# ethz-asl/laser_slam

Measured on AMD Instinct MI355X. Metric: scans_per_sec, higher is better.
Workload: dtype f32

## Files before the change

laser_slam_amd/csrc/lsgpu_icp.hip:

```cpp
#include <cstring>
#include <cmath>
#include <cstdio>
#include <cstdlib>
#include <string>
#include <vector>
#include <chrono>
#include <system_error>
#include <thread>
#include <utility>

#include <dlfcn.h>

#include <hip/hip_runtime.h>
#include <rccl/rccl.h>

#include "../../include/lsgpu_icp.h"
#include "lsgpu_grid.hip.h"
#include "lsgpu_tuning.h"
#include "lsgpu_policy.h"
#include "lsgpu_knn.hip.h"
#include "lsgpu_knn_k.hip.h"
#include "lsgpu_snf.hip.h"
#include "lsgpu_max_density.hip.h"
#include "lsgpu_cone.hip.h"
// ... 218 lines not shown
  DevBuf<double> amb_val;

  DevBuf<SsnSeg> ssn_seg_a, ssn_seg_b;
  DevBuf<int> ssn_axis_a, ssn_axis_b;
  DevBuf<uint32_t> ssn_seg_fb;
  DevBuf<SegBlock> ssn_blocktab;
  DevBuf<uint32_t> ssn_seg_of, ssn_box_pts, ssn_box_base, ssn_keep, ssn_out_pos, ssn_bb, ssn_bounds_ws;
  DevBuf<float> ssn_box_normal, ssn_draws;
  DevBuf<uint32_t> gs_e[2], gs_k[6];
  DevBuf<GsBlock> gs_tab;
  DevBuf<GsSegBlocks> gs_sblk;
  DevBuf<uint32_t> gs_hist;
  DevBuf<GsMedian> gs_cand, gs_median;
  DevBuf<uint32_t> gs_cand_blk, gs_cand_n, gs_cl, gs_err;
  DevBuf<uint2> gs_rng;
  uint32_t* h_gs_err = nullptr;
  int64_t gs_plan_n = -1;
  int gs_plan_levels = -1;
  std::vector<uint32_t> gs_lvl_first, gs_lvl_blocks;
  DevBuf<float4> flt_in, flt_in2, flt_ref, flt_rd;
  DevBuf<float4> vgf_out;
  DevBuf<float> flt_nrm;
  bool cuts_on = false;
  lsgpu_chain_cuts cuts{};
  DevBuf<uint32_t> cut_blk;
  DevBuf<float4> cut_ref;
  bool md_on = false;
  lsgpu_max_density_config md_cfg{};
  DevBuf<float> dens, dens_io;
  DevBuf<MdStat> md_stat;
// ... 335 lines not shown
  for (auto& e : h->knn_events) { (void)hipEventDestroy(e.a); (void)hipEventDestroy(e.b); (void)hipEventDestroy(e.c); (void)hipEventDestroy(e.d); (void)hipEventDestroy(e.e); }
  if (h->ev0) (void)hipEventDestroy(h->ev0);
  if (h->ev1) (void)hipEventDestroy(h->ev1);
  if (h->ev_state) (void)hipEventDestroy(h->ev_state);
  if (h->ev_tail) (void)hipEventDestroy(h->ev_tail);
  if (h->cone_done) (void)hipEventDestroy(h->cone_done);
  if (h->cone_occ_ready) (void)hipEventDestroy(h->cone_occ_ready);
  for (auto& e : h->ev_pay) if (e) (void)hipEventDestroy(e);
  if (h->pin) (void)hipHostFree(h->pin);
  if (h->h_price) (void)hipHostFree(h->h_price);
  if (h->h_cone_occ) (void)hipHostFree(h->h_cone_occ);
  if (h->h_gs_err) (void)hipHostFree(h->h_gs_err);
  for (auto& bf : h->gs_e) bf.release();
  for (auto& bf : h->gs_k) bf.release();
  h->gs_tab.release(); h->gs_sblk.release(); h->gs_hist.release(); h->gs_cand.release(); h->gs_median.release();
  h->gs_cand_blk.release(); h->gs_cand_n.release(); h->gs_cl.release(); h->gs_err.release(); h->gs_rng.release();
  if (h->draws_pinned) (void)hipHostFree(h->draws_pinned);
  if (h->copy_done) (void)hipEventDestroy(h->copy_done);
  if (h->ref_up_done) (void)hipEventDestroy(h->ref_up_done);
  if (h->draws_done) (void)hipEventDestroy(h->draws_done);
  if (h->draws_first_done) (void)hipEventDestroy(h->draws_first_done);
  if (h->draw_stream) { (void)hipStreamSynchronize(h->draw_stream); (void)hipStreamDestroy(h->draw_stream); }
  if (h->side_done) (void)hipEventDestroy(h->side_done);
  if (h->side_stream) { (void)hipStreamSynchronize(h->side_stream); (void)hipStreamDestroy(h->side_stream); }
  if (h->copy_stream) (void)hipStreamDestroy(h->copy_stream);
  if (h->stream) (void)hipStreamDestroy(h->stream);
  delete h;
}

}

// ... 1131 lines not shown
        HIPC(hipMemcpyAsync(h->gs_tab.p, tab.data(), tab.size() * sizeof(GsBlock), hipMemcpyHostToDevice, h->stream));
        HIPC(hipMemcpyAsync(h->gs_sblk.p, sblk.data(), sblk.size() * sizeof(GsSegBlocks), hipMemcpyHostToDevice, h->stream));
        HIPC(hipStreamSynchronize(h->stream));
      }
      h->gs_plan_n = n; h->gs_plan_levels = glevels;
    }
    const size_t nseg_g = (size_t)1 << glevels;
    int cap = 1;
    for (uint32_t v : h->gs_lvl_blocks) cap = std::max(cap, (int)v);
    for (auto& bf : h->gs_e) HIPC(bf.reserve(n));
    for (auto& bf : h->gs_k) HIPC(bf.reserve(n));
    HIPC(h->gs_hist.reserve(4 * 256 * (nseg_g + 1))); HIPC(h->gs_median.reserve(nseg_g)); HIPC(h->gs_cand_n.reserve(2 * nseg_g + 2));
    const size_t cand_room = std::max<size_t>(nseg_g / 2, 1) * kGsCandRoom;
    HIPC(h->gs_cand.reserve(cand_room)); HIPC(h->gs_cand_blk.reserve(cand_room));
    HIPC(h->gs_cl.reserve((size_t)2 * cap)); HIPC(h->gs_err.reserve(8)); HIPC(h->gs_rng.reserve(2 * nseg_g + 2));
    HIPC(h->ssn_axis_a.reserve(nseg_g)); HIPC(h->ssn_axis_b.reserve(nseg_g));
    if (!h->h_gs_err) HIPC(hipHostMalloc((void**)&h->h_gs_err, 64, hipHostMallocDefault));
    uint32_t* cand_n[2] = {h->gs_cand_n.p, h->gs_cand_n.p + nseg_g + 1};
    uint32_t* sig_cur = reinterpret_cast<uint32_t*>(h->ssn_axis_a.p);
    uint32_t* sig_nxt = reinterpret_cast<uint32_t*>(h->ssn_axis_b.p);
    GsSet in, out;
    in.e = h->gs_e[0].p; out.e = h->gs_e[1].p;
    for (int d = 0; d < 3; ++d) { in.k[d] = h->gs_k[d].p; out.k[d] = h->gs_k[3 + d].p; }
    uint2* rng_cur = h->gs_rng.p;
    uint2* rng_nxt = h->gs_rng.p + nseg_g + 1;
    uint32_t* gh1[2] = {h->gs_hist.p, h->gs_hist.p + 256 * (nseg_g + 1)};
    uint32_t* gh2[2] = {h->gs_hist.p + 2 * 256 * (nseg_g + 1), h->gs_hist.p + 3 * 256 * (nseg_g + 1)};
    hipLaunchKernelGGL(k_gs_init, dim3(nblk(n)), dim3(256), 0, h->stream, src, (int)n, in, out.e, (const SsnSeg*)cur, (const uint32_t*)h->ssn_bb.p, rng_cur,
                       gh1[0], gh2[0], cand_n[0], sig_cur, h->gs_err.p);
    for (int L = 0; L < glevels; ++L) {
      const int ns = 1 << L, nb = (int)h->gs_lvl_blocks[L], par = L & 1;
      const GsBlock* tab = h->gs_tab.p + h->gs_lvl_first[L];
      const GsSegBlocks* sblk = h->gs_sblk.p + (ns - 1);
      hipLaunchKernelGGL(k_gs_hist<1>, dim3(nb), dim3(256), 0, h->stream, tab, cur, (const uint2*)rng_cur, in, gh1[par], gh2[par], h->gs_err.p);
      hipLaunchKernelGGL(k_gs_hist<2>, dim3(nb), dim3(256), 0, h->stream, tab, cur, (const uint2*)rng_cur, in, gh1[par], gh2[par], h->gs_err.p);
      const uint32_t lvl_cap = (uint32_t)std::min<size_t>(cand_room / (size_t)ns, (size_t)1 << 22);
      hipLaunchKernelGGL(k_gs_collect, dim3(nb), dim3(256), 0, h->stream, tab, cur, (const uint2*)rng_cur, (const uint32_t*)sig_cur, in,
                         (const uint32_t*)gh1[par], (const uint32_t*)gh2[par], cand_n[par], h->gs_cand.p, h->gs_cand_blk.p, lvl_cap, h->gs_cl.p);
      hipLaunchKernelGGL(k_gs_select, dim3(ns), dim3(L < 3 ? 1024 : 256), 0, h->stream, sblk, src, cur, (const uint32_t*)sig_cur, gh1[par], gh2[par],
                         gh1[par ^ 1], gh2[par ^ 1], cand_n[par], (const GsMedian*)h->gs_cand.p, (const uint32_t*)h->gs_cand_blk.p, lvl_cap, h->gs_cl.p,
                         h->gs_cl.p + cap, h->gs_median.p, nxt, sig_nxt, cand_n[par ^ 1], rng_nxt, h->gs_err.p);
      hipLaunchKernelGGL(k_gs_part, dim3(nb), dim3(kGsPartThreads), 0, h->stream, tab, cur, (const uint32_t*)sig_cur, in, out,
                         (const GsMedian*)h->gs_median.p, (const uint32_t*)(h->gs_cl.p + cap), (const SsnSeg*)nxt, rng_nxt, h->gs_err.p);
      std::swap(in, out);
      std::swap(cur, nxt);
      std::swap(sig_cur, sig_nxt);
      std::swap(rng_cur, rng_nxt);
    }
    idx = in.e;
    root_sig = sig_cur;
    HIPC(hipGetLastError());
  } else if (glevels > 0) {
    const size_t nseg_g = (size_t)1 << glevels;
    const int cap = (int)(n / kSegTile + (int64_t)(nseg_g / 2) + 2);
    HIPC(h->lane.scratch->vals_alt.reserve(n));
    HIPC(h->ssn_axis_a.reserve(nseg_g)); HIPC(h->ssn_axis_b.reserve(nseg_g)); HIPC(h->ssn_seg_fb.reserve(nseg_g));
    HIPC(h->ssn_blocktab.reserve((size_t)cap)); HIPC(h->lane.scratch->sort_hist.reserve((size_t)256 * cap + 256 + 4));
    uint32_t* keyA = reinterpret_cast<uint32_t*>(h->lane.scratch->keys.p);
    uint32_t* keyB = keyA + n;
// ... 38 lines not shown
    uint32_t* idx_rw = const_cast<uint32_t*>(idx);
    if (root_max == 8192)
      hipLaunchKernelGGL(k_ssn_tree<8192>, dim3(1 << glevels), dim3(1024), 0, h->stream, src, idx_rw, cur, knn, levels - glevels, h->ssn_seg_of.p, nxt, root_axis, root_sig);
    else if (root_max == 4096)
      hipLaunchKernelGGL(k_ssn_tree<4096>, dim3(1 << glevels), dim3(512), 0, h->stream, src, idx_rw, cur, knn, levels - glevels, h->ssn_seg_of.p, nxt, root_axis, root_sig);
    else
      hipLaunchKernelGGL(k_ssn_tree<2048>, dim3(1 << glevels), dim3(256), 0, h->stream, src, idx_rw, cur, knn, levels - glevels, h->ssn_seg_of.p, nxt, root_axis, root_sig);
    std::swap(cur, nxt);
  }
  if (levels == 0) {
    hipLaunchKernelGGL(k_ssn_keys, dim3(nblk(n)), dim3(256), 0, h->stream, src, (int)n, (const uint32_t*)nullptr,
                       (const uint32_t*)nullptr, cur, knn, h->lane.scratch->keys.p, h->lane.scratch->vals.p);
    HIPC(hipMemsetAsync(h->ssn_seg_of.p, 0, (size_t)n * 4, h->stream));
    idx = h->lane.scratch->vals.p;
  }
  hipLaunchKernelGGL(k_ssn_boxes, dim3((int)((nseg + 127) / 128)), dim3(128), 0, h->stream, src, idx, cur, (int)nseg,
                     h->ssn_box_normal.p, h->ssn_box_pts.p);
  HIPC(hipGetLastError());
  int rc = scan_u32(h, h->ssn_box_pts.p, h->ssn_box_base.p, nseg);
  if (rc) return rc;
  rc = ahead->ready(first_draw + (size_t)n);
  if (rc) return rc;
  hipLaunchKernelGGL(k_ssn_select, dim3(nblk(n)), dim3(256), 0, h->stream, (int)n, idx, h->ssn_seg_of.p, cur,
                     h->ssn_box_pts.p, h->ssn_box_base.p, h->ssn_draws.p + first_draw, ratio, h->ssn_keep.p);
  rc = scan_u32(h, h->ssn_keep.p, h->ssn_out_pos.p, (size_t)n, false,  true);
  if (rc == LSGPU_OK) {
    hipLaunchKernelGGL(k_ssn_emit, dim3(nblk(n)), dim3(256), 0, h->stream, src, (int)n,
                       h->ssn_box_normal.p, h->ssn_keep.p, h->ssn_out_pos.p, out_xyz1, out_nrm);
  }
  uint32_t n_draws = 0, kept = 0;
  if (rc == LSGPU_OK)
    rc = scan_totals(h, h->ssn_box_pts.p, h->ssn_box_base.p, nseg, h->ssn_keep.p, h->ssn_out_pos.p, (size_t)n, &n_draws, &kept,
// ... 1624 lines not shown
```

laser_slam_amd/csrc/lsgpu_ssn.hip.h:

```cpp
#pragma once
#include "lsgpu_common.hip.h"
#include "lsgpu_box_normal.h"
#include "lsgpu_segsort.hip.h"
#include "lsgpu_chain_cut.hip.h"

namespace lsgpu {

struct SsnSeg {
  uint32_t start, count;
  float lo[3], hi[3];
};
constexpr int kSsnMaxKnn = 32;

__device__ __forceinline__ uint32_t float_order_key(float f) {
  uint32_t u = __float_as_uint(f);
  if (u == 0x80000000u) u = 0u;
  return (u & 0x80000000u) ? ~u : (u | 0x80000000u);
}
__device__ __forceinline__ float float_from_order_key(uint32_t k) {
  return __uint_as_float((k & 0x80000000u) ? (k & 0x7FFFFFFFu) : ~k);
}

__device__ __forceinline__ float coord_of(const float4& p, int d) { return d == 0 ? p.x : (d == 1 ? p.y : p.z); }

// ... 237 lines not shown
  const SsnSeg sg = segs[s];
  uint32_t kept = 0;
  if (sg.count > 0) {
    float n[3];
    const uint32_t* bi = idx + sg.start;
    if (boxnormal::box_normal((int)sg.count, [&](int i, int d) { return coord_of(p[bi[i]], d); }, n)) {
      kept = sg.count;
      box_normal[3 * (size_t)s + 0] = n[0];
      box_normal[3 * (size_t)s + 1] = n[1];
      box_normal[3 * (size_t)s + 2] = n[2];
    }
  }
  box_pts[s] = kept;
}

__global__ __launch_bounds__(256) void k_ssn_select(int n, const uint32_t* __restrict__ idx,
                                                    const uint32_t* __restrict__ seg_of,
                                                    const SsnSeg* __restrict__ segs,
                                                    const uint32_t* __restrict__ box_pts,
                                                    const uint32_t* __restrict__ box_base,
                                                    const float* __restrict__ draws, float ratio,
                                                    uint32_t* __restrict__ keep) {
  const int pos = blockIdx.x * 256 + threadIdx.x;
  if (pos >= n) return;
  const uint32_t s = seg_of[pos];
  uint32_t k = 0;
  if (box_pts[s]) {
    const float r = draws[box_base[s] + ((uint32_t)pos - segs[s].start)];
    k = r < ratio ? 1u : 0u;
  }
// ... 138 lines not shown
```

laser_slam_amd/csrc/lsgpu_ssn_select.hip.h:

```cpp
#pragma once
#include "lsgpu_ssn.hip.h"
#include "lsgpu_ssn_tree.hip.h"

namespace lsgpu {

#ifdef LSGPU_KNN_STATS
#define LSGPU_SEL_T(n) do { if (gridDim.x == 1 && threadIdx.x == 0) g_tree_dbg[n] = (unsigned long long)clock64(); } while (0)
#else
#define LSGPU_SEL_T(n) do { } while (0)
#endif

constexpr uint32_t kGsTile = 2048u;
constexpr int kGsPartThreads = 512;
constexpr uint32_t kGsCandCap = 2048u;
constexpr uint32_t kGsCandRoom = 16384u;
constexpr uint32_t kGsNoAxis = 0xFFu;
constexpr uint32_t kGsSelBlocks = 8192u;

struct GsSet {
  uint32_t* e;
  uint32_t* k[3];
};
__device__ __forceinline__ uint32_t* gs_k(const GsSet& g, int d) { return d == 0 ? g.k[0] : d == 1 ? g.k[1] : g.k[2]; }

struct GsBlock {
  uint32_t first, count;
  uint32_t seg;
  uint32_t seg_start, seg_count;
  uint32_t fb, nb;
  uint32_t pad;
};
struct GsSegBlocks { uint32_t fb, nb, start, count; };

struct GsMedian { uint32_t ka, k1, k2, e; };

__host__ __device__ __forceinline__ uint32_t gs_sig_push(uint32_t sig, uint32_t a) {
  const uint32_t o1 = sig & 0xFFu, o2 = (sig >> 8) & 0xFFu, o3 = (sig >> 16) & 0xFFu;
  if (o1 == a) return sig;
  const uint32_t r2 = o2 == a ? o3 : o2;
  return a | (o1 << 8) | (r2 << 16) | 0xFF000000u;
}
__device__ __forceinline__ void gs_other_axes(uint32_t sig, uint32_t a, uint32_t& x1, uint32_t& x2) {
  const uint32_t o1 = sig & 0xFFu, o2 = (sig >> 8) & 0xFFu, o3 = (sig >> 16) & 0xFFu;
  if (o1 == a) { x1 = o2; x2 = o3; }
  else { x1 = o1; x2 = o2 == a ? o3 : o2; }
}
__device__ __forceinline__ bool gs_less(uint32_t ka, uint32_t k1, uint32_t k2, uint32_t e, const GsMedian& m) {
  return ka != m.ka ? ka < m.ka : k1 != m.k1 ? k1 < m.k1 : k2 != m.k2 ? k2 < m.k2 : e < m.e;
}
// ... 32 lines not shown
  const uint32_t total = fbs[ns];
  for (uint32_t sg = threadIdx.x; sg < ns; sg += 1024u)
    sblk[(ns - 1u) + sg] = GsSegBlocks{fbs[sg], fbs[sg + 1u] - fbs[sg], sc[sg].x, sc[sg].y};
  GsBlock* __restrict__ t = tab + lvl.first[L];
  for (uint32_t j = threadIdx.x; j < total; j += 1024u) {
    uint32_t lo = 0u, hi = ns;
    while (hi - lo > 1u) { const uint32_t mid = (lo + hi) >> 1; if (fbs[mid] <= j) lo = mid; else hi = mid; }
    const uint32_t k = j - fbs[lo], st = sc[lo].x, c = sc[lo].y;
    const uint32_t off = k * kGsTile;
    t[j] = GsBlock{st + off, min(kGsTile, c - off), lo, st, c, fbs[lo], fbs[lo + 1u] - fbs[lo], 0u};
  }
}

__global__ __launch_bounds__(256) void k_gs_init(const float4* __restrict__ p, int n, GsSet out, uint32_t* __restrict__ other_e,
                                                 const SsnSeg* __restrict__ root, const uint32_t* __restrict__ bb,
                                                 uint2* __restrict__ rng, uint32_t* __restrict__ gh1_root,
                                                 uint32_t* __restrict__ gh2_root, uint32_t* __restrict__ cand_n_root,
                                                 uint32_t* __restrict__ sig_root, uint32_t* __restrict__ err) {
  const int i = blockIdx.x * 256 + threadIdx.x;
  if (blockIdx.x == 0) {
    gh1_root[threadIdx.x] = 0u; gh2_root[threadIdx.x] = 0u;
    if (threadIdx.x < 8) err[threadIdx.x] = 0u;
    if (threadIdx.x == 0) {
      const int a = ssn_cut_axis(root[0]); rng[0] = make_uint2(bb[a], bb[3 + a]);
      cand_n_root[0] = 0u; sig_root[0] = 0xFFFFFFFFu;
    }
  }
  if (i >= n) return;
  const float4 v = p[i];
  out.e[i] = (uint32_t)i; other_e[i] = (uint32_t)i;
  out.k[0][i] = float_order_key(v.x); out.k[1][i] = float_order_key(v.y); out.k[2][i] = float_order_key(v.z);
}

struct GsCut { int a; uint32_t klo, khi; float xlo, scale; };
__device__ __forceinline__ GsCut gs_cut(const SsnSeg& sg, const uint2 rng ) {
  GsCut c;
  c.a = ssn_cut_axis(sg);
  c.klo = rng.x; c.khi = rng.y >= rng.x ? rng.y : rng.x;
  c.xlo = float_from_order_key(c.klo);
  const float ext = float_from_order_key(c.khi) - c.xlo;
  c.scale = ext > 0.f ? 65536.0f / ext : 0.f;
  return c;
}
__device__ __forceinline__ uint32_t gs_bin16(const GsCut& c, uint32_t k) {
  const float t = (float_from_order_key(k) - c.xlo) * c.scale;
  return (uint32_t)fminf(fmaxf(t, 0.f), 65535.f);
}

__device__ __forceinline__ void gs_find_bin(const uint32_t* __restrict__ gh, uint32_t target, uint32_t* sh ,
                                            uint32_t& bin, uint32_t& below) {
  const int lane = threadIdx.x & 63, w = threadIdx.x >> 6;
  const bool act = threadIdx.x < 256u;
  const uint32_t tot = act ? gh[threadIdx.x] : 0u;
  const uint32_t incl = wave_scan_incl_u32(tot, lane);
  if (threadIdx.x == 0) { sh[4] = 0xFFFFFFFFu; sh[5] = 0u; }
  if (act && lane == 63) sh[w] = incl;
  __syncthreads();
  uint32_t before = 0u;
  for (int ww = 0; ww < w && ww < 4; ++ww) before += sh[ww];
  const uint32_t excl = before + incl - tot;
  if (act && tot != 0u && excl <= target && target < excl + tot) { sh[4] = threadIdx.x; sh[5] = excl; }
  __syncthreads();
  bin = sh[4]; below = sh[5];
  __syncthreads();
}

template <int PASS>
__global__ __launch_bounds__(256) void k_gs_hist(const GsBlock* __restrict__ tab, const SsnSeg* __restrict__ segs,
                                                 const uint2* __restrict__ rng, GsSet in, uint32_t* __restrict__ gh1,
                                                 uint32_t* __restrict__ gh2, uint32_t* __restrict__ err) {
  __shared__ uint32_t hist[256];
  __shared__ uint32_t sh[8];
  hist[threadIdx.x] = 0u;
  const GsBlock sb = tab[blockIdx.x];
  const GsCut c = gs_cut(segs[sb.seg], rng[sb.seg]);
  const uint32_t* __restrict__ ka = gs_k(in, c.a);
  uint32_t mb1 = 0u, below1 = 0u;
  if (PASS == 2) gs_find_bin(gh1 + (size_t)sb.seg * 256u, sb.seg_count - sb.seg_count / 2u, sh, mb1, below1);
  else __syncthreads();
  bool bad = PASS == 2 && mb1 == 0xFFFFFFFFu;
  for (uint32_t j = threadIdx.x; j < sb.count; j += 256u) {
    const uint32_t k = ka[sb.first + j];
    bad = bad || k < c.klo || k > c.khi;
    const uint32_t b16 = gs_bin16(c, k), b1 = b16 >> 8;
    if (PASS == 1) atomicAdd(&hist[b1], 1u);
    else if (b1 == mb1) atomicAdd(&hist[b16 & 255u], 1u);
  }
  if (bad) { err[0] = 1u; err[1] = 1u; err[2] = sb.seg; }
  __syncthreads();
  const uint32_t v = hist[threadIdx.x];
  if (v) atomicAdd(&(PASS == 1 ? gh1 : gh2)[(size_t)sb.seg * 256u + threadIdx.x], v);
}

__global__ __launch_bounds__(256) void k_gs_collect(const GsBlock* __restrict__ tab, const SsnSeg* __restrict__ segs,
                                                    const uint2* __restrict__ rng,
                                                    const uint32_t* __restrict__ sig, GsSet in, const uint32_t* __restrict__ gh1,
                                                    const uint32_t* __restrict__ gh2,
                                                    uint32_t* __restrict__ cand_n, GsMedian* __restrict__ cand,
                                                    uint32_t* __restrict__ cand_blk, uint32_t cap ,
                                                    uint32_t* __restrict__ cl) {
  __shared__ uint32_t ws[4];
  __shared__ uint32_t sh[8];
  const GsBlock sb = tab[blockIdx.x];
  const GsCut c = gs_cut(segs[sb.seg], rng[sb.seg]);
  const uint32_t leftn = sb.seg_count - sb.seg_count / 2u;
  uint32_t mb1, below1, mb2, below2;
  gs_find_bin(gh1 + (size_t)sb.seg * 256u, leftn, sh, mb1, below1);
  gs_find_bin(gh2 + (size_t)sb.seg * 256u, leftn - below1, sh, mb2, below2);
  uint32_t x1, x2;
  gs_other_axes(sig[sb.seg], (uint32_t)c.a, x1, x2);
  const uint32_t* __restrict__ ka = gs_k(in, c.a);
  uint32_t left = 0u;
  const int lane = threadIdx.x & 63;
  for (uint32_t j0 = 0; j0 < sb.count; j0 += 256u) {
    const uint32_t j = j0 + threadIdx.x;
    const bool live = j < sb.count;
    const uint32_t i = sb.first + (live ? j : 0u);
    const uint32_t k = live ? ka[i] : 0u;
    const uint32_t b16 = gs_bin16(c, k), b1 = b16 >> 8, b2 = b16 & 255u;
    const bool is_cand = live && b1 == mb1 && b2 == mb2;
    if (live && (b1 < mb1 || (b1 == mb1 && b2 < mb2))) ++left;
    const unsigned long long m = __ballot(is_cand);
    if (m != 0ull) {
      uint32_t base = 0u;
      if (lane == 0) base = atomicAdd(&cand_n[sb.seg], (uint32_t)__popcll(m));
      base = (uint32_t)__shfl((int)base, 0);
      const uint32_t slot = base + (uint32_t)__popcll(m & ((1ull << lane) - 1ull));
      if (is_cand && slot < cap) {
        GsMedian md;
        md.ka = k; md.e = in.e[i];
        md.k1 = x1 != kGsNoAxis ? gs_k(in, (int)x1)[i] : 0u;
        md.k2 = x2 != kGsNoAxis ? gs_k(in, (int)x2)[i] : 0u;
        cand[(size_t)sb.seg * cap + slot] = md;
        cand_blk[(size_t)sb.seg * cap + slot] = blockIdx.x;
// ... 3 lines not shown
  left = wave_sum_u32(left);
  if ((threadIdx.x & 63) == 0) ws[threadIdx.x >> 6] = left;
  __syncthreads();
  if (threadIdx.x == 0) cl[blockIdx.x] = ws[0] + ws[1] + ws[2] + ws[3];
}

__global__ __launch_bounds__(1024) void k_gs_select(const GsSegBlocks* __restrict__ sblk, const float4* __restrict__ p,
                                                   const SsnSeg* __restrict__ segs, const uint32_t* __restrict__ sig,
                                                   uint32_t* __restrict__ gh1, uint32_t* __restrict__ gh2,
                                                   uint32_t* __restrict__ gh1_next, uint32_t* __restrict__ gh2_next,
                                                   uint32_t* __restrict__ cand_n,
                                                   const GsMedian* __restrict__ cand, const uint32_t* __restrict__ cand_blk, uint32_t cap,
                                                   uint32_t* __restrict__ cl, uint32_t* __restrict__ clp, GsMedian* __restrict__ median,
                                                   SsnSeg* __restrict__ out, uint32_t* __restrict__ sig_out,
                                                   uint32_t* __restrict__ cand_n_next, uint2* __restrict__ rng_next,
                                                   uint32_t* __restrict__ err) {
  __shared__ GsMedian lc[kGsCandCap];
  __shared__ uint32_t med_slot;
  __shared__ GsMedian med_sh;
  __shared__ uint32_t sh[8];
  __shared__ uint32_t rh[256];
  __shared__ uint32_t lcnt[kGsSelBlocks];
  __shared__ uint32_t lblk[kGsCandCap];
  LSGPU_SEL_T(48);
  const uint32_t s = blockIdx.x;
  const GsSegBlocks q = sblk[s];
  const uint32_t n = cand_n[s];
  const uint32_t left = q.count - q.count / 2u;
  uint32_t mb1, below1, mb2, below2;
  gs_find_bin(gh1 + (size_t)s * 256u, left, sh, mb1, below1);
  gs_find_bin(gh2 + (size_t)s * 256u, left - below1, sh, mb2, below2);
  const uint32_t target = left - below1 - below2;
  LSGPU_SEL_T(49);
  if (threadIdx.x < 256u) {
    gh1_next[(size_t)(2u * s) * 256u + threadIdx.x] = 0u; gh1_next[(size_t)(2u * s + 1u) * 256u + threadIdx.x] = 0u;
    gh2_next[(size_t)(2u * s) * 256u + threadIdx.x] = 0u; gh2_next[(size_t)(2u * s + 1u) * 256u + threadIdx.x] = 0u;
  }
  if (threadIdx.x == 0) {
    med_slot = 0xFFFFFFFFu;
    cand_n_next[2u * s] = 0u; cand_n_next[2u * s + 1u] = 0u;
    rng_next[2u * s] = make_uint2(0xFFFFFFFFu, 0u); rng_next[2u * s + 1u] = make_uint2(0xFFFFFFFFu, 0u);
    if (n > cap || target >= n || mb1 == 0xFFFFFFFFu || mb2 == 0xFFFFFFFFu) { err[0] = 1u; err[1] = 3u; err[2] = s; err[3] = n; err[4] = target; }
  }
  const uint32_t c = min(n, cap);
  const GsMedian* __restrict__ gc = cand + (size_t)s * cap;
  const uint32_t* __restrict__ gb = cand_blk + (size_t)s * cap;
  const bool in_lds = c <= kGsCandCap;
  const bool lds_counts = q.nb <= kGsSelBlocks;
  if (lds_counts) for (uint32_t b = threadIdx.x; b < q.nb; b += blockDim.x) lcnt[b] = 0u;
  if (in_lds) for (uint32_t i = threadIdx.x; i < c; i += blockDim.x) { lc[i] = gc[i]; lblk[i] = gb[i]; }
  __syncthreads();
  LSGPU_SEL_T(50);
#ifdef LSGPU_KNN_STATS
  if (gridDim.x == 1 && threadIdx.x == 0) g_tree_dbg[54] = c;
#endif
  uint32_t arrived = 0u;
// ... 94 lines not shown
    median[s] = m;
    const SsnSeg sg = segs[s];
    const int cut = ssn_cut_axis(sg);
    SsnSeg a = sg, b = sg;
    const float cutval = have ? coord_of(p[m.e], cut) : coord_of(make_float4(sg.hi[0], sg.hi[1], sg.hi[2], 0.f), cut);
#pragma unroll
    for (int d = 0; d < 3; ++d) {
      a.hi[d] = d == cut ? cutval : a.hi[d];
      b.lo[d] = d == cut ? cutval : b.lo[d];
    }
    a.start = q.start; a.count = left;
    b.start = q.start + left; b.count = q.count - left;
    out[2u * s] = a; out[2u * s + 1u] = b;
    const uint32_t sv = gs_sig_push(sig[s], (uint32_t)cut);
    sig_out[2u * s] = sv; sig_out[2u * s + 1u] = sv;
  }
  LSGPU_SEL_T(53);
}

__global__ __launch_bounds__(kGsPartThreads) void k_gs_part(const GsBlock* __restrict__ tab, const SsnSeg* __restrict__ segs,
                                                 const uint32_t* __restrict__ sig, GsSet in, GsSet out,
                                                 const GsMedian* __restrict__ median, const uint32_t* __restrict__ clp,
                                                 const SsnSeg* __restrict__ segs_next, uint2* __restrict__ rng_next,
                                                 uint32_t* __restrict__ err) {
  constexpr int kW = kGsPartThreads / 64, kI = (int)kGsTile / kGsPartThreads;
  __shared__ uint32_t ws[kW];
  __shared__ uint32_t rr[kW][4];
  __shared__ uint32_t stage[4][kGsTile];
  const int lane = threadIdx.x & 63, w = threadIdx.x >> 6;
  const GsBlock sb = tab[blockIdx.x];
  const SsnSeg sg = segs[sb.seg];
  const int a = ssn_cut_axis(sg);
  uint32_t x1, x2;
  gs_other_axes(sig[sb.seg], (uint32_t)a, x1, x2);
  const GsMedian m = median[sb.seg];
  const uint32_t base_left = clp[blockIdx.x];
  const uint32_t left_total = sb.seg_count - sb.seg_count / 2u;
  const uint32_t base_right = (sb.first - sb.seg_start) - base_left;
  uint32_t ev[kI], kx[kI], ky[kI], kz[kI], xl[kI];
  uint32_t carry = 0u;
  const int aL = ssn_cut_axis(segs_next[2u * sb.seg]), aR = ssn_cut_axis(segs_next[2u * sb.seg + 1u]);
  uint32_t mnL = 0xFFFFFFFFu, mxL = 0u, mnR = 0xFFFFFFFFu, mxR = 0u;
#pragma unroll
  for (int k = 0; k < kI; ++k) {
    const uint32_t j = (uint32_t)(w * (64 * kI) + k * 64 + lane);
    uint32_t v = 0u;
    ev[k] = kx[k] = ky[k] = kz[k] = 0u;
    if (j < sb.count) {
      const uint32_t i = sb.first + j;
      ev[k] = in.e[i]; kx[k] = in.k[0][i]; ky[k] = in.k[1][i]; kz[k] = in.k[2][i];
      const uint32_t ka = a == 0 ? kx[k] : a == 1 ? ky[k] : kz[k];
      const uint32_t k1 = x1 == kGsNoAxis ? 0u : x1 == 0u ? kx[k] : x1 == 1u ? ky[k] : kz[k];
      const uint32_t k2 = x2 == kGsNoAxis ? 0u : x2 == 0u ? kx[k] : x2 == 1u ? ky[k] : kz[k];
      v = gs_less(ka, k1, k2, ev[k], m) ? 1u : 0u;
      if (v) { const uint32_t kc = aL == 0 ? kx[k] : aL == 1 ? ky[k] : kz[k]; mnL = min(mnL, kc); mxL = max(mxL, kc); }
      else   { const uint32_t kc = aR == 0 ? kx[k] : aR == 1 ? ky[k] : kz[k]; mnR = min(mnR, kc); mxR = max(mxR, kc); }
    }
    const uint32_t incl = tree_wave_scan(v, lane);
    xl[k] = ((carry + incl - v) << 1) | v;
    carry += rl_u(incl, 63);
  }
  __syncthreads();
  mnL = ~wave_max_u32(~mnL); mxL = wave_max_u32(mxL); mnR = ~wave_max_u32(~mnR); mxR = wave_max_u32(mxR);
  if (lane == 0) { ws[w] = carry; rr[w][0] = mnL; rr[w][1] = mxL; rr[w][2] = mnR; rr[w][3] = mxR; }
  __syncthreads();
  if (threadIdx.x < 4) {
    const int q = (int)threadIdx.x;
    const bool is_min = (q & 1) == 0;
    uint32_t v = rr[0][q];
    for (int ww = 1; ww < kW; ++ww) v = is_min ? min(v, rr[ww][q]) : max(v, rr[ww][q]);
    uint32_t* word = reinterpret_cast<uint32_t*>(&rng_next[2u * sb.seg + (uint32_t)(q >> 1)]) + (q & 1);
    const uint32_t seen = __hip_atomic_load(word, __ATOMIC_RELAXED, __HIP_MEMORY_SCOPE_AGENT);
    if (is_min ? v < seen : v > seen) { if (is_min) atomicMin(word, v); else atomicMax(word, v); }
  }
  uint32_t before = 0u;
  for (int ww = 0; ww < w; ++ww) before += ws[ww];
  uint32_t nleft = 0u;
  for (int ww = 0; ww < kW; ++ww) nleft += ws[ww];
#pragma unroll
  for (int k = 0; k < kI; ++k) {
    const uint32_t j = (uint32_t)(w * (64 * kI) + k * 64 + lane);
    if (j < sb.count) {
      const uint32_t lbefore = before + (xl[k] >> 1);
      const uint32_t slot = (xl[k] & 1u) ? lbefore : nleft + (j - lbefore);
      stage[0][slot] = ev[k]; stage[1][slot] = kx[k]; stage[2][slot] = ky[k]; stage[3][slot] = kz[k];
    }
  }
  __syncthreads();
  const uint32_t dst_left = sb.seg_start + base_left, dst_right = sb.seg_start + left_total + base_right;
  const uint32_t pos0 = sb.first - sb.seg_start;
  const bool bad = base_left > pos0 || base_left + nleft > left_total ||
                   (pos0 - base_left) + (sb.count - nleft) > sb.seg_count - left_total;
  if (bad) {
    if (threadIdx.x == 0) { err[0] = 1u; err[5] = 4u; err[6] = sb.seg; err[7] = dst_left; }
    for (uint32_t t = threadIdx.x; t < sb.count; t += (uint32_t)kGsPartThreads) {
      const uint32_t d = sb.first + t;
      out.e[d] = stage[0][t]; out.k[0][d] = stage[1][t]; out.k[1][d] = stage[2][t]; out.k[2][d] = stage[3][t];
    }
    return;
  }
#pragma unroll
  for (int k = 0; k < kI; ++k) {
    const uint32_t t = (uint32_t)(k * kGsPartThreads) + threadIdx.x;
    if (t < sb.count) {
      const uint32_t d = t < nleft ? dst_left + t : dst_right + (t - nleft);
      out.e[d] = stage[0][t]; out.k[0][d] = stage[1][t]; out.k[1][d] = stage[2][t]; out.k[2][d] = stage[3][t];
    }
  }
}

}
```

Measured before the change: 253.1.

## Fuse first-pass histogram into partition and stage box-normal points in LDS

The median-split partition kernel now also builds the next level's coarse histogram and tracks the 3-axis extents of each child. This removes the separate k_gs_hist<1> launch and read pass on every level after the first. The second-pass histogram uses the tightened extent range to rebin the candidate coarse bin, and child key ranges are now set from parent extents in the select kernel. Separately, box-normal estimation gets an LDS-staged variant that gathers each block's points once when the neighbourhood size is small. The cost is more registers, shared memory and atomics in the partition kernel.

```diff
diff --git a/laser_slam_amd/csrc/lsgpu_icp.hip b/laser_slam_amd/csrc/lsgpu_icp.hip
--- a/laser_slam_amd/csrc/lsgpu_icp.hip
+++ b/laser_slam_amd/csrc/lsgpu_icp.hip
@@ -256,6 +256,7 @@
   DevBuf<GsMedian> gs_cand, gs_median;
   DevBuf<uint32_t> gs_cand_blk, gs_cand_n, gs_cl, gs_err;
   DevBuf<uint2> gs_rng;
+  DevBuf<GsRange3> gs_xr;
   uint32_t* h_gs_err = nullptr;
   int64_t gs_plan_n = -1;
   int gs_plan_levels = -1;
@@ -621,7 +622,7 @@
   for (auto& bf : h->gs_e) bf.release();
   for (auto& bf : h->gs_k) bf.release();
   h->gs_tab.release(); h->gs_sblk.release(); h->gs_hist.release(); h->gs_cand.release(); h->gs_median.release();
-  h->gs_cand_blk.release(); h->gs_cand_n.release(); h->gs_cl.release(); h->gs_err.release(); h->gs_rng.release();
+  h->gs_cand_blk.release(); h->gs_cand_n.release(); h->gs_cl.release(); h->gs_err.release(); h->gs_rng.release(); h->gs_xr.release();
   if (h->draws_pinned) (void)hipHostFree(h->draws_pinned);
   if (h->copy_done) (void)hipEventDestroy(h->copy_done);
   if (h->ref_up_done) (void)hipEventDestroy(h->ref_up_done);
@@ -1783,6 +1784,7 @@
     const size_t cand_room = std::max<size_t>(nseg_g / 2, 1) * kGsCandRoom;
     HIPC(h->gs_cand.reserve(cand_room)); HIPC(h->gs_cand_blk.reserve(cand_room));
     HIPC(h->gs_cl.reserve((size_t)2 * cap)); HIPC(h->gs_err.reserve(8)); HIPC(h->gs_rng.reserve(2 * nseg_g + 2));
+    HIPC(h->gs_xr.reserve(2 * nseg_g + 2));
     HIPC(h->ssn_axis_a.reserve(nseg_g)); HIPC(h->ssn_axis_b.reserve(nseg_g));
     if (!h->h_gs_err) HIPC(hipHostMalloc((void**)&h->h_gs_err, 64, hipHostMallocDefault));
     uint32_t* cand_n[2] = {h->gs_cand_n.p, h->gs_cand_n.p + nseg_g + 1};
@@ -1795,23 +1797,27 @@
     uint2* rng_nxt = h->gs_rng.p + nseg_g + 1;
     uint32_t* gh1[2] = {h->gs_hist.p, h->gs_hist.p + 256 * (nseg_g + 1)};
     uint32_t* gh2[2] = {h->gs_hist.p + 2 * 256 * (nseg_g + 1), h->gs_hist.p + 3 * 256 * (nseg_g + 1)};
+    GsRange3* xr_cur = h->gs_xr.p;
+    GsRange3* xr_nxt = h->gs_xr.p + nseg_g + 1;
     hipLaunchKernelGGL(k_gs_init, dim3(nblk(n)), dim3(256), 0, h->stream, src, (int)n, in, out.e, (const SsnSeg*)cur, (const uint32_t*)h->ssn_bb.p, rng_cur,
-                       gh1[0], gh2[0], cand_n[0], sig_cur, h->gs_err.p);
+                       xr_cur, gh1[0], gh2[0], cand_n[0], sig_cur, h->gs_err.p);
     for (int L = 0; L < glevels; ++L) {
       const int ns = 1 << L, nb = (int)h->gs_lvl_blocks[L], par = L & 1;
       const GsBlock* tab = h->gs_tab.p + h->gs_lvl_first[L];
       const GsSegBlocks* sblk = h->gs_sblk.p + (ns - 1);
-      hipLaunchKernelGGL(k_gs_hist<1>, dim3(nb), dim3(256), 0, h->stream, tab, cur, (const uint2*)rng_cur, in, gh1[par], gh2[par], h->gs_err.p);
-      hipLaunchKernelGGL(k_gs_hist<2>, dim3(nb), dim3(256), 0, h->stream, tab, cur, (const uint2*)rng_cur, in, gh1[par], gh2[par], h->gs_err.p);
+      if (L == 0) hipLaunchKernelGGL(k_gs_hist<1>, dim3(nb), dim3(256), 0, h->stream, tab, cur, (const uint2*)rng_cur, (const GsRange3*)xr_cur, in, gh1[par], gh2[par], h->gs_err.p);
+      hipLaunchKernelGGL(k_gs_hist<2>, dim3(nb), dim3(256), 0, h->stream, tab, cur, (const uint2*)rng_cur, (const GsRange3*)xr_cur, in, gh1[par], gh2[par], h->gs_err.p);
       const uint32_t lvl_cap = (uint32_t)std::min<size_t>(cand_room / (size_t)ns, (size_t)1 << 22);
-      hipLaunchKernelGGL(k_gs_collect, dim3(nb), dim3(256), 0, h->stream, tab, cur, (const uint2*)rng_cur, (const uint32_t*)sig_cur, in,
+      hipLaunchKernelGGL(k_gs_collect, dim3(nb), dim3(256), 0, h->stream, tab, cur, (const uint2*)rng_cur, (const GsRange3*)xr_cur, (const uint32_t*)sig_cur, in,
                          (const uint32_t*)gh1[par], (const uint32_t*)gh2[par], cand_n[par], h->gs_cand.p, h->gs_cand_blk.p, lvl_cap, h->gs_cl.p);
       hipLaunchKernelGGL(k_gs_select, dim3(ns), dim3(L < 3 ? 1024 : 256), 0, h->stream, sblk, src, cur, (const uint32_t*)sig_cur, gh1[par], gh2[par],
                          gh1[par ^ 1], gh2[par ^ 1], cand_n[par], (const GsMedian*)h->gs_cand.p, (const uint32_t*)h->gs_cand_blk.p, lvl_cap, h->gs_cl.p,
-                         h->gs_cl.p + cap, h->gs_median.p, nxt, sig_nxt, cand_n[par ^ 1], rng_nxt, h->gs_err.p);
+                         h->gs_cl.p + cap, h->gs_median.p, nxt, sig_nxt, cand_n[par ^ 1], rng_nxt, (const GsRange3*)xr_cur, xr_nxt, h->gs_err.p);
       hipLaunchKernelGGL(k_gs_part, dim3(nb), dim3(kGsPartThreads), 0, h->stream, tab, cur, (const uint32_t*)sig_cur, in, out,
-                         (const GsMedian*)h->gs_median.p, (const uint32_t*)(h->gs_cl.p + cap), (const SsnSeg*)nxt, rng_nxt, h->gs_err.p);
+                         (const GsMedian*)h->gs_median.p, (const uint32_t*)(h->gs_cl.p + cap), (const SsnSeg*)nxt, (const uint2*)rng_nxt, xr_nxt,
+                         L + 1 < glevels ? gh1[par ^ 1] : (uint32_t*)nullptr, h->gs_err.p);
       std::swap(in, out);
+      std::swap(xr_cur, xr_nxt);
       std::swap(cur, nxt);
       std::swap(sig_cur, sig_nxt);
       std::swap(rng_cur, rng_nxt);
@@ -1880,8 +1886,12 @@
     HIPC(hipMemsetAsync(h->ssn_seg_of.p, 0, (size_t)n * 4, h->stream));
     idx = h->lane.scratch->vals.p;
   }
-  hipLaunchKernelGGL(k_ssn_boxes, dim3((int)((nseg + 127) / 128)), dim3(128), 0, h->stream, src, idx, cur, (int)nseg,
-                     h->ssn_box_normal.p, h->ssn_box_pts.p);
+  if (knn <= kSsnBoxStage)
+    hipLaunchKernelGGL(k_ssn_boxes_staged, dim3((int)((nseg + 127) / 128)), dim3(128), 0, h->stream, src, idx, cur, (int)nseg,
+                       h->ssn_box_normal.p, h->ssn_box_pts.p);
+  else
+    hipLaunchKernelGGL(k_ssn_boxes, dim3((int)((nseg + 127) / 128)), dim3(128), 0, h->stream, src, idx, cur, (int)nseg,
+                       h->ssn_box_normal.p, h->ssn_box_pts.p);
   HIPC(hipGetLastError());
   int rc = scan_u32(h, h->ssn_box_pts.p, h->ssn_box_base.p, nseg);
   if (rc) return rc;
diff --git a/laser_slam_amd/csrc/lsgpu_ssn.hip.h b/laser_slam_amd/csrc/lsgpu_ssn.hip.h
--- a/laser_slam_amd/csrc/lsgpu_ssn.hip.h
+++ b/laser_slam_amd/csrc/lsgpu_ssn.hip.h
@@ -275,6 +275,66 @@
   box_pts[s] = kept;
 }
 
+constexpr int kSsnBoxStage = 16;
+__global__ __launch_bounds__(128) void k_ssn_boxes_staged(const float4* __restrict__ p, const uint32_t* __restrict__ idx,
+                                                          const SsnSeg* __restrict__ segs, int nseg,
+                                                          float* __restrict__ box_normal, uint32_t* __restrict__ box_pts) {
+  constexpr uint32_t kRoom = 128u * kSsnBoxStage;
+  __shared__ float sx[kRoom], sy[kRoom], sz[kRoom];
+  __shared__ uint32_t range[2];
+  const int s = blockIdx.x * 128 + threadIdx.x;
+  SsnSeg sg;
+  sg.start = 0u; sg.count = 0u;
+  if (s < nseg) sg = segs[s];
+  if (threadIdx.x == 0) { range[0] = 0xFFFFFFFFu; range[1] = 0u; }
+  __syncthreads();
+  if (sg.count > 0) { atomicMin(&range[0], sg.start); atomicMax(&range[1], sg.start + sg.count); }
+  __syncthreads();
+  const uint32_t begin = range[0], end = range[1];
+  const bool staged = begin < end && end - begin <= kRoom;
+  if (staged) {
+    const uint32_t total = end - begin;
+    uint32_t id[kSsnBoxStage];
+    float4 v[kSsnBoxStage];
+#pragma unroll
+    for (int u = 0; u < kSsnBoxStage; ++u) {
+      const uint32_t t = (uint32_t)(u * 128) + threadIdx.x;
+      id[u] = t < total ? idx[begin + t] : 0u;
+    }
+#pragma unroll
+    for (int u = 0; u < kSsnBoxStage; ++u) {
+      const uint32_t t = (uint32_t)(u * 128) + threadIdx.x;
+      if (t < total) v[u] = p[id[u]];
+    }
+#pragma unroll
+    for (int u = 0; u < kSsnBoxStage; ++u) {
+      const uint32_t t = (uint32_t)(u * 128) + threadIdx.x;
+      if (t < total) { sx[t] = v[u].x; sy[t] = v[u].y; sz[t] = v[u].z; }
+    }
+  }
+  __syncthreads();
+  if (s >= nseg) return;
+  uint32_t kept = 0;
+  if (sg.count > 0) {
+    float n[3];
+    bool ok;
+    if (staged) {
+      const uint32_t o = sg.start - begin;
+      ok = boxnormal::box_normal((int)sg.count, [&](int i, int d) { return d == 0 ? sx[o + i] : (d == 1 ? sy[o + i] : sz[o + i]); }, n);
+    } else {
+      const uint32_t* bi = idx + sg.start;
+      ok = boxnormal::box_normal((int)sg.count, [&](int i, int d) { return coord_of(p[bi[i]], d); }, n);
+    }
+    if (ok) {
+      kept = sg.count;
+      box_normal[3 * (size_t)s + 0] = n[0];
+      box_normal[3 * (size_t)s + 1] = n[1];
+      box_normal[3 * (size_t)s + 2] = n[2];
+    }
+  }
+  box_pts[s] = kept;
+}
+
 __global__ __launch_bounds__(256) void k_ssn_select(int n, const uint32_t* __restrict__ idx,
                                                     const uint32_t* __restrict__ seg_of,
                                                     const SsnSeg* __restrict__ segs,
diff --git a/laser_slam_amd/csrc/lsgpu_ssn_select.hip.h b/laser_slam_amd/csrc/lsgpu_ssn_select.hip.h
--- a/laser_slam_amd/csrc/lsgpu_ssn_select.hip.h
+++ b/laser_slam_amd/csrc/lsgpu_ssn_select.hip.h
@@ -33,6 +33,7 @@
 struct GsSegBlocks { uint32_t fb, nb, start, count; };
 
 struct GsMedian { uint32_t ka, k1, k2, e; };
+struct GsRange3 { uint32_t w[6]; };
 
 __host__ __device__ __forceinline__ uint32_t gs_sig_push(uint32_t sig, uint32_t a) {
   const uint32_t o1 = sig & 0xFFu, o2 = (sig >> 8) & 0xFFu, o3 = (sig >> 16) & 0xFFu;
@@ -95,13 +96,14 @@
 
 __global__ __launch_bounds__(256) void k_gs_init(const float4* __restrict__ p, int n, GsSet out, uint32_t* __restrict__ other_e,
                                                  const SsnSeg* __restrict__ root, const uint32_t* __restrict__ bb,
-                                                 uint2* __restrict__ rng, uint32_t* __restrict__ gh1_root,
+                                                 uint2* __restrict__ rng, GsRange3* __restrict__ xr, uint32_t* __restrict__ gh1_root,
                                                  uint32_t* __restrict__ gh2_root, uint32_t* __restrict__ cand_n_root,
                                                  uint32_t* __restrict__ sig_root, uint32_t* __restrict__ err) {
   const int i = blockIdx.x * 256 + threadIdx.x;
   if (blockIdx.x == 0) {
     gh1_root[threadIdx.x] = 0u; gh2_root[threadIdx.x] = 0u;
     if (threadIdx.x < 8) err[threadIdx.x] = 0u;
+    if (threadIdx.x < 6) xr[0].w[threadIdx.x] = bb[threadIdx.x];
     if (threadIdx.x == 0) {
       const int a = ssn_cut_axis(root[0]); rng[0] = make_uint2(bb[a], bb[3 + a]);
       cand_n_root[0] = 0u; sig_root[0] = 0xFFFFFFFFu;
@@ -128,6 +130,22 @@
   return (uint32_t)fminf(fmaxf(t, 0.f), 65535.f);
 }
 
+struct GsCut2 { float xlo, scale; };
+__device__ __forceinline__ GsCut2 gs_cut2(const GsCut& c, uint32_t mb1, const GsRange3& xr) {
+  const float w1 = c.scale > 0.f ? 256.0f / c.scale : 0.f;
+  const uint32_t elo = c.a == 0 ? xr.w[0] : c.a == 1 ? xr.w[1] : xr.w[2], ehi = c.a == 0 ? xr.w[3] : c.a == 1 ? xr.w[4] : xr.w[5];
+  const float lo = fmaxf(c.xlo + (float)mb1 * w1, float_from_order_key(elo));
+  const float hi = fminf(c.xlo + ((float)mb1 + 1.0f) * w1, float_from_order_key(ehi));
+  GsCut2 r;
+  r.xlo = lo;
+  r.scale = hi - lo > 0.f ? 256.0f / (hi - lo) : 0.f;
+  return r;
+}
+__device__ __forceinline__ uint32_t gs_bin8(const GsCut2& c, uint32_t k) {
+  const float t = (float_from_order_key(k) - c.xlo) * c.scale;
+  return (uint32_t)fminf(fmaxf(t, 0.f), 255.f);
+}
+
 __device__ __forceinline__ void gs_find_bin(const uint32_t* __restrict__ gh, uint32_t target, uint32_t* sh ,
                                             uint32_t& bin, uint32_t& below) {
   const int lane = threadIdx.x & 63, w = threadIdx.x >> 6;
@@ -148,24 +166,27 @@
 
 template <int PASS>
 __global__ __launch_bounds__(256) void k_gs_hist(const GsBlock* __restrict__ tab, const SsnSeg* __restrict__ segs,
-                                                 const uint2* __restrict__ rng, GsSet in, uint32_t* __restrict__ gh1,
-                                                 uint32_t* __restrict__ gh2, uint32_t* __restrict__ err) {
+                                                 const uint2* __restrict__ rng, const GsRange3* __restrict__ xr, GsSet in,
+                                                 uint32_t* __restrict__ gh1, uint32_t* __restrict__ gh2, uint32_t* __restrict__ err) {
   __shared__ uint32_t hist[256];
   __shared__ uint32_t sh[8];
   hist[threadIdx.x] = 0u;
   const GsBlock sb = tab[blockIdx.x];
   const GsCut c = gs_cut(segs[sb.seg], rng[sb.seg]);
+  const GsRange3 xs = xr[sb.seg];
   const uint32_t* __restrict__ ka = gs_k(in, c.a);
   uint32_t mb1 = 0u, below1 = 0u;
   if (PASS == 2) gs_find_bin(gh1 + (size_t)sb.seg * 256u, sb.seg_count - sb.seg_count / 2u, sh, mb1, below1);
   else __syncthreads();
   bool bad = PASS == 2 && mb1 == 0xFFFFFFFFu;
+  GsCut2 c2{0.f, 0.f};
+  if (PASS == 2) c2 = gs_cut2(c, mb1, xs);
   for (uint32_t j = threadIdx.x; j < sb.count; j += 256u) {
     const uint32_t k = ka[sb.first + j];
     bad = bad || k < c.klo || k > c.khi;
     const uint32_t b16 = gs_bin16(c, k), b1 = b16 >> 8;
     if (PASS == 1) atomicAdd(&hist[b1], 1u);
-    else if (b1 == mb1) atomicAdd(&hist[b16 & 255u], 1u);
+    else if (b1 == mb1) atomicAdd(&hist[gs_bin8(c2, k)], 1u);
   }
   if (bad) { err[0] = 1u; err[1] = 1u; err[2] = sb.seg; }
   __syncthreads();
@@ -174,7 +195,7 @@
 }
 
 __global__ __launch_bounds__(256) void k_gs_collect(const GsBlock* __restrict__ tab, const SsnSeg* __restrict__ segs,
-                                                    const uint2* __restrict__ rng,
+                                                    const uint2* __restrict__ rng, const GsRange3* __restrict__ xr,
                                                     const uint32_t* __restrict__ sig, GsSet in, const uint32_t* __restrict__ gh1,
                                                     const uint32_t* __restrict__ gh2,
                                                     uint32_t* __restrict__ cand_n, GsMedian* __restrict__ cand,
@@ -184,10 +205,12 @@
   __shared__ uint32_t sh[8];
   const GsBlock sb = tab[blockIdx.x];
   const GsCut c = gs_cut(segs[sb.seg], rng[sb.seg]);
+  const GsRange3 xs = xr[sb.seg];
   const uint32_t leftn = sb.seg_count - sb.seg_count / 2u;
   uint32_t mb1, below1, mb2, below2;
   gs_find_bin(gh1 + (size_t)sb.seg * 256u, leftn, sh, mb1, below1);
   gs_find_bin(gh2 + (size_t)sb.seg * 256u, leftn - below1, sh, mb2, below2);
+  const GsCut2 c2 = gs_cut2(c, mb1, xs);
   uint32_t x1, x2;
   gs_other_axes(sig[sb.seg], (uint32_t)c.a, x1, x2);
   const uint32_t* __restrict__ ka = gs_k(in, c.a);
@@ -198,7 +221,7 @@
     const bool live = j < sb.count;
     const uint32_t i = sb.first + (live ? j : 0u);
     const uint32_t k = live ? ka[i] : 0u;
-    const uint32_t b16 = gs_bin16(c, k), b1 = b16 >> 8, b2 = b16 & 255u;
+    const uint32_t b1 = gs_bin16(c, k) >> 8, b2 = gs_bin8(c2, k);
     const bool is_cand = live && b1 == mb1 && b2 == mb2;
     if (live && (b1 < mb1 || (b1 == mb1 && b2 < mb2))) ++left;
     const unsigned long long m = __ballot(is_cand);
@@ -232,6 +255,7 @@
                                                    uint32_t* __restrict__ cl, uint32_t* __restrict__ clp, GsMedian* __restrict__ median,
                                                    SsnSeg* __restrict__ out, uint32_t* __restrict__ sig_out,
                                                    uint32_t* __restrict__ cand_n_next, uint2* __restrict__ rng_next,
+                                                   const GsRange3* __restrict__ xr, GsRange3* __restrict__ xr_next,
                                                    uint32_t* __restrict__ err) {
   __shared__ GsMedian lc[kGsCandCap];
   __shared__ uint32_t med_slot;
@@ -243,6 +267,7 @@
   LSGPU_SEL_T(48);
   const uint32_t s = blockIdx.x;
   const GsSegBlocks q = sblk[s];
+  const GsRange3 pr = xr[s];
   const uint32_t n = cand_n[s];
   const uint32_t left = q.count - q.count / 2u;
   uint32_t mb1, below1, mb2, below2;
@@ -254,10 +279,11 @@
     gh1_next[(size_t)(2u * s) * 256u + threadIdx.x] = 0u; gh1_next[(size_t)(2u * s + 1u) * 256u + threadIdx.x] = 0u;
     gh2_next[(size_t)(2u * s) * 256u + threadIdx.x] = 0u; gh2_next[(size_t)(2u * s + 1u) * 256u + threadIdx.x] = 0u;
   }
+  if (threadIdx.x < 12u)
+    xr_next[2u * s + (threadIdx.x >= 6u ? 1u : 0u)].w[threadIdx.x % 6u] = (threadIdx.x % 6u) < 3u ? 0xFFFFFFFFu : 0u;
   if (threadIdx.x == 0) {
     med_slot = 0xFFFFFFFFu;
     cand_n_next[2u * s] = 0u; cand_n_next[2u * s + 1u] = 0u;
-    rng_next[2u * s] = make_uint2(0xFFFFFFFFu, 0u); rng_next[2u * s + 1u] = make_uint2(0xFFFFFFFFu, 0u);
     if (n > cap || target >= n || mb1 == 0xFFFFFFFFu || mb2 == 0xFFFFFFFFu) { err[0] = 1u; err[1] = 3u; err[2] = s; err[3] = n; err[4] = target; }
   }
   const uint32_t c = min(n, cap);
@@ -382,6 +408,11 @@
     out[2u * s] = a; out[2u * s + 1u] = b;
     const uint32_t sv = gs_sig_push(sig[s], (uint32_t)cut);
     sig_out[2u * s] = sv; sig_out[2u * s + 1u] = sv;
+    const int aL = ssn_cut_axis(a), aR = ssn_cut_axis(b);
+    const uint32_t loL = aL == 0 ? pr.w[0] : aL == 1 ? pr.w[1] : pr.w[2], hiL = aL == 0 ? pr.w[3] : aL == 1 ? pr.w[4] : pr.w[5];
+    const uint32_t loR = aR == 0 ? pr.w[0] : aR == 1 ? pr.w[1] : pr.w[2], hiR = aR == 0 ? pr.w[3] : aR == 1 ? pr.w[4] : pr.w[5];
+    rng_next[2u * s] = make_uint2(loL, have && aL == cut ? m.ka : hiL);
+    rng_next[2u * s + 1u] = make_uint2(have && aR == cut ? m.ka : loR, hiR);
   }
   LSGPU_SEL_T(53);
 }
@@ -389,11 +420,14 @@
 __global__ __launch_bounds__(kGsPartThreads) void k_gs_part(const GsBlock* __restrict__ tab, const SsnSeg* __restrict__ segs,
                                                  const uint32_t* __restrict__ sig, GsSet in, GsSet out,
                                                  const GsMedian* __restrict__ median, const uint32_t* __restrict__ clp,
-                                                 const SsnSeg* __restrict__ segs_next, uint2* __restrict__ rng_next,
+                                                 const SsnSeg* __restrict__ segs_next, const uint2* __restrict__ rng_next,
+                                                 GsRange3* __restrict__ xr_next, uint32_t* __restrict__ gh1_next ,
                                                  uint32_t* __restrict__ err) {
   constexpr int kW = kGsPartThreads / 64, kI = (int)kGsTile / kGsPartThreads;
   __shared__ uint32_t ws[kW];
-  __shared__ uint32_t rr[kW][4];
+  __shared__ uint32_t rr[kW][12];
+  __shared__ uint32_t ch[2][256];
+  static_assert(kGsPartThreads == 512, "k_gs_part: one thread per child and bin flushes the histograms");
   __shared__ uint32_t stage[4][kGsTile];
   const int lane = threadIdx.x & 63, w = threadIdx.x >> 6;
   const GsBlock sb = tab[blockIdx.x];
@@ -407,8 +441,11 @@
   const uint32_t base_right = (sb.first - sb.seg_start) - base_left;
   uint32_t ev[kI], kx[kI], ky[kI], kz[kI], xl[kI];
   uint32_t carry = 0u;
-  const int aL = ssn_cut_axis(segs_next[2u * sb.seg]), aR = ssn_cut_axis(segs_next[2u * sb.seg + 1u]);
-  uint32_t mnL = 0xFFFFFFFFu, mxL = 0u, mnR = 0xFFFFFFFFu, mxR = 0u;
+  const bool hist = gh1_next != nullptr;
+  const GsCut cL = gs_cut(segs_next[2u * sb.seg], rng_next[2u * sb.seg]), cR = gs_cut(segs_next[2u * sb.seg + 1u], rng_next[2u * sb.seg + 1u]);
+  if (hist) { ch[0][threadIdx.x & 255u] = 0u; ch[1][threadIdx.x & 255u] = 0u; }
+  uint32_t mn[2][3] = {{0xFFFFFFFFu, 0xFFFFFFFFu, 0xFFFFFFFFu}, {0xFFFFFFFFu, 0xFFFFFFFFu, 0xFFFFFFFFu}}, mx[2][3] = {{0u, 0u, 0u}, {0u, 0u, 0u}};
+  __syncthreads();
 #pragma unroll
   for (int k = 0; k < kI; ++k) {
     const uint32_t j = (uint32_t)(w * (64 * kI) + k * 64 + lane);
@@ -421,23 +458,38 @@
       const uint32_t k1 = x1 == kGsNoAxis ? 0u : x1 == 0u ? kx[k] : x1 == 1u ? ky[k] : kz[k];
       const uint32_t k2 = x2 == kGsNoAxis ? 0u : x2 == 0u ? kx[k] : x2 == 1u ? ky[k] : kz[k];
       v = gs_less(ka, k1, k2, ev[k], m) ? 1u : 0u;
-      if (v) { const uint32_t kc = aL == 0 ? kx[k] : aL == 1 ? ky[k] : kz[k]; mnL = min(mnL, kc); mxL = max(mxL, kc); }
-      else   { const uint32_t kc = aR == 0 ? kx[k] : aR == 1 ? ky[k] : kz[k]; mnR = min(mnR, kc); mxR = max(mxR, kc); }
+      if (v) {
+        mn[0][0] = min(mn[0][0], kx[k]); mn[0][1] = min(mn[0][1], ky[k]); mn[0][2] = min(mn[0][2], kz[k]);
+        mx[0][0] = max(mx[0][0], kx[k]); mx[0][1] = max(mx[0][1], ky[k]); mx[0][2] = max(mx[0][2], kz[k]);
+      } else {
+        mn[1][0] = min(mn[1][0], kx[k]); mn[1][1] = min(mn[1][1], ky[k]); mn[1][2] = min(mn[1][2], kz[k]);
+        mx[1][0] = max(mx[1][0], kx[k]); mx[1][1] = max(mx[1][1], ky[k]); mx[1][2] = max(mx[1][2], kz[k]);
+      }
+      if (hist) {
+        const int ac = v ? cL.a : cR.a;
+        const uint32_t kc = ac == 0 ? kx[k] : ac == 1 ? ky[k] : kz[k];
+        atomicAdd(&ch[v ? 0 : 1][gs_bin16(v ? cL : cR, kc) >> 8], 1u);
+      }
     }
     const uint32_t incl = tree_wave_scan(v, lane);
     xl[k] = ((carry + incl - v) << 1) | v;
     carry += rl_u(incl, 63);
   }
-  __syncthreads();
-  mnL = ~wave_max_u32(~mnL); mxL = wave_max_u32(mxL); mnR = ~wave_max_u32(~mnR); mxR = wave_max_u32(mxR);
-  if (lane == 0) { ws[w] = carry; rr[w][0] = mnL; rr[w][1] = mxL; rr[w][2] = mnR; rr[w][3] = mxR; }
-  __syncthreads();
-  if (threadIdx.x < 4) {
+#pragma unroll
+  for (int sd = 0; sd < 2; ++sd)
+#pragma unroll
+    for (int d = 0; d < 3; ++d) {
+      const uint32_t lo = ~wave_max_u32(~mn[sd][d]), hi = wave_max_u32(mx[sd][d]);
+      if (lane == 0) { rr[w][6 * sd + d] = lo; rr[w][6 * sd + 3 + d] = hi; }
+    }
+  if (lane == 0) ws[w] = carry;
+  __syncthreads();
+  if (threadIdx.x < 12) {
     const int q = (int)threadIdx.x;
-    const bool is_min = (q & 1) == 0;
+    const bool is_min = q % 6 < 3;
     uint32_t v = rr[0][q];
     for (int ww = 1; ww < kW; ++ww) v = is_min ? min(v, rr[ww][q]) : max(v, rr[ww][q]);
-    uint32_t* word = reinterpret_cast<uint32_t*>(&rng_next[2u * sb.seg + (uint32_t)(q >> 1)]) + (q & 1);
+    uint32_t* word = &xr_next[2u * sb.seg + (uint32_t)(q / 6)].w[q % 6];
     const uint32_t seen = __hip_atomic_load(word, __ATOMIC_RELAXED, __HIP_MEMORY_SCOPE_AGENT);
     if (is_min ? v < seen : v > seen) { if (is_min) atomicMin(word, v); else atomicMax(word, v); }
   }
@@ -467,6 +519,10 @@
     }
     return;
   }
+  if (hist) {
+    const uint32_t v = ch[threadIdx.x >> 8][threadIdx.x & 255u];
+    if (v) atomicAdd(&gh1_next[(size_t)(2u * sb.seg + (threadIdx.x >> 8)) * 256u + (threadIdx.x & 255u)], v);
+  }
 #pragma unroll
   for (int k = 0; k < kI; ++k) {
     const uint32_t t = (uint32_t)(k * kGsPartThreads) + threadIdx.x;
```

Result: no change. 252.9 (-0.1%).
